# MLCogUP/nspeech

Measured on AMD Instinct MI355X. Metric: mel-frames/sec Tacotron-2 LJSpeech bs32 train step, higher is better.
Workload: dtype bf16; 1 GPU; Tacotron-2 train step (fwd+bwd+clip+Adam), batch 32/GPU, T_in 160, T_out 1000, r=5; targets = spectrogram features of synthetic speech (SURVEY 8d); global_batch=32, parallelism=dp1, deterministic_gradients=True

## Files before the change

include/nspeech_hip.h:

```cpp
#ifndef NSPEECH_HIP_H
#define NSPEECH_HIP_H
#include <stddef.h>
#include <stdint.h>

#ifdef __cplusplus
extern "C" {
#endif

typedef void* ns_stream_t;

enum { NS_OK = 0, NS_ERR_BAD_ARG = -1, NS_ERR_UNSUPPORTED_SHAPE = -2, NS_ERR_LAUNCH = -3,
       NS_ERR_SHORT_BUFFER = -4  };
enum { NS_F32 = 0, NS_BF16 = 1, NS_F64 = 2  };
enum { NS_ACT_NONE = 0, NS_ACT_RELU = 1, NS_ACT_TANH = 2, NS_ACT_SIGMOID = 3,
       NS_ACT_SOFTSIGN = 4  };

int ns_version(void);
const char* ns_device_arch(void);
const char* ns_last_error(void);

int ns_occupy(int blocks, int threads, int lds_bytes, int heavy, double usec, int* started, ns_stream_t stream);
int ns_wait_counter(const int* counter, int target, double timeout_usec, ns_stream_t stream);

typedef struct {
// ... 181 lines not shown
  int reverse;
  float forget_bias;
  void* h; int64_t ld_h;
  float* c;
  void* gates;
  const float* dh; int64_t ld_dh;
  void* dgates;
  float* work;
  int f32_passes;
  const void* whT_hi; const void* whT_lo; const void* wh_bf16;
  void* dgates_bf16;
  void* h_bf16; int64_t ld_h_bf16;
  uint32_t zoneout_thr_cell, zoneout_thr_output;
  uint32_t zoneout_seed_cell, zoneout_seed_output;
  float cell_clip;
} ns_lstm_seq_params;
int ns_lstm_seq_fwd(const ns_lstm_seq_params* p, ns_stream_t stream);
int ns_lstm_seq_bwd(const ns_lstm_seq_params* p, ns_stream_t stream);
size_t ns_lstm_seq_work_bytes(const ns_lstm_seq_params* p);
int ns_lstm_seq2_fwd(const ns_lstm_seq_params* p0, const ns_lstm_seq_params* p1, ns_stream_t stream);
int ns_lstm_seq2_bwd(const ns_lstm_seq_params* p0, const ns_lstm_seq_params* p1, ns_stream_t stream);


int ns_lstm_cluster_supported(const ns_lstm_seq_params* fw, const ns_lstm_seq_params* bw, int backward);
size_t ns_lstm_cluster_work_bytes(const ns_lstm_seq_params* p);
int ns_lstm_cluster_fwd(const ns_lstm_seq_params* fw, const ns_lstm_seq_params* bw, void* work, ns_stream_t stream);
int ns_lstm_cluster_bwd(const ns_lstm_seq_params* fw, const ns_lstm_seq_params* bw, void* work, ns_stream_t stream);

int ns_lstm_wide_supported(const ns_lstm_seq_params* p, int backward);
size_t ns_lstm_wide_work_bytes(const ns_lstm_seq_params* p);
// ... 369 lines not shown
```

nspeech_amd/csrc/lstm_wide.hip:

```cpp
#include "common.h"
#include <stdint.h>
#include <stdlib.h>

namespace {
constexpr int WT = 512, WW = WT / 64;
typedef unsigned int u32x4 __attribute__((ext_vector_type(4)));
constexpr size_t WIDE_TRACE_BYTES = 256 * 8 * sizeof(long long);

struct WideArgs {
  ns_lstm_seq_params p;
  int* status;
  long long* trace;
  int nub;
};
__device__ __forceinline__ void wstamp(const WideArgs& a, int st, int k) {
  if (a.trace && blockIdx.x == 0 && threadIdx.x == 0 && st < 256) a.trace[st * 8 + k] = wall_clock64();
}

template <typename T> __device__ __forceinline__ bool has_sentinel(const u32x4& v);
template <> __device__ __forceinline__ bool has_sentinel<float>(const u32x4& v) {
  return (v[0] == 0xffffffffu) | (v[1] == 0xffffffffu) | (v[2] == 0xffffffffu) | (v[3] == 0xffffffffu);
}
template <> __device__ __forceinline__ bool has_sentinel<bf16_t>(const u32x4& v) {
  bool b = false;
#pragma unroll
  for (int i = 0; i < 4; ++i) b = b | ((v[i] & 0xffffu) == 0xffffu) | (v[i] >= 0xffff0000u);
  return b;
}
__device__ __forceinline__ float clean(float x, float*) { return __float_as_uint(x) == 0xffffffffu ? __uint_as_float(0x7fc00000u) : x; }
__device__ __forceinline__ bf16_t clean(float x, bf16_t*) {
  const bf16_t b = (bf16_t)x;
  return __builtin_bit_cast(unsigned short, b) == 0xffffu ? __builtin_bit_cast(bf16_t, (unsigned short)0x7fc0u) : b;
}

template <typename T>
__global__ __launch_bounds__(256) void wide_fill_kernel(T* base, int N, long P, int padl, int T_, long ld, int width) {
  const int ppr = width * (int)sizeof(T) / 16;
  const long total = (long)N * T_ * ppr;
  const u32x4 s = {0xffffffffu, 0xffffffffu, 0xffffffffu, 0xffffffffu};
  for (long i = (long)blockIdx.x * blockDim.x + threadIdx.x; i < total; i += (long)gridDim.x * blockDim.x) {
    const long row = i / ppr;
    const int pc = (int)(i - row * ppr);
// ... 21 lines not shown
      ready |= __builtin_amdgcn_ballot_w64(lane < NP && !has_sentinel<T>(pv));
      if (tslot && ready == ALLP && blockIdx.x == 0 && threadIdx.x == 0) *tslot = wall_clock64();
    }
#pragma unroll
    for (int l = 0; l < NL; ++l) {
      constexpr unsigned long long one = 1ull;
      const unsigned long long m = ((one << PPCH) - one) << ((l / LPC) * PPCH);
      if (!(done & (1u << l)) && (ready & m) == m) {
        const unsigned o = off0 + (unsigned)(l % LPC) * in_grp + (unsigned)(l / LPC) * per_grp;
        v[l] = __builtin_amdgcn_raw_buffer_load_b128(rs, o, 0, 16);
        done |= 1u << l;
      }
    }
    ++spins;
    if (done == ALLL) {
      unsigned stale = 0u;
#pragma unroll
      for (int l = 0; l < NL; ++l) if (__any(has_sentinel<T>(v[l]))) stale |= 1u << l;
      if (!stale) return spins;
      done &= ~stale;
    }
    if ((spins & 255u) == 0) {
      if (__hip_atomic_load(status, __ATOMIC_RELAXED, __HIP_MEMORY_SCOPE_AGENT)) { if (lane == 0) *abortf = 1; return 0; }
      if ((spins & 1023u) == 0 && ns_spin_timed_out(clk0)) { if (lane == 0) { atomicExch(status, code); *abortf = 1; } return 0; }
    }
  }
}

constexpr int WTF = WT + 128;
template <typename T, int PASSES, int NCH>
__global__ __launch_bounds__(WTF) void lstm_wide_fwd_kernel(WideArgs a) {
  __shared__ float red[2][WW][16][36];
  __shared__ __attribute__((aligned(16))) T hst[16][8];
  __shared__ int abortf;
  const ns_lstm_seq_params& p = a.p;
  const int tid = threadIdx.x, lane = tid & 63, wave = __builtin_amdgcn_readfirstlane(tid >> 6);
  const int H = p.H, NUB = a.nub;
  const int rg = blockIdx.x / NUB, ub = blockIdx.x % NUB;
  const int n0 = rg * 16, u0 = ub * 8;
  if (tid == 0) abortf = 0;
  const size_t hbytes = (size_t)p.N * p.P * p.ld_h * sizeof(T);
  constexpr int PPC = 8 * (int)sizeof(T) / 16;
  __syncthreads();

  if (wave < WW) {
    const int r16 = lane & 15, g = lane >> 4;
    const int k0 = wave * (H / WW);
    bf16x8 bh[2][NCH], bl[2][NCH];
#pragma unroll
    for (int j = 0; j < 2; ++j) {
      const long wrow = ((long)(2 * j + (r16 >> 3)) * H + u0 + (r16 & 7)) * H + k0 + g * 8;
#pragma unroll
      for (int c = 0; c < NCH; ++c) {
        if constexpr (PASSES == 3) {
          bh[j][c] = *(const bf16x8*)((const bf16_t*)p.whT_hi + wrow + c * 32);
          bl[j][c] = *(const bf16x8*)((const bf16_t*)p.whT_lo + wrow + c * 32);
        } else {
          bh[j][c] = *(const bf16x8*)((const bf16_t*)p.whT + wrow + c * 32);
          bl[j][c] = bh[j][c];
        }
      }
    }
    const bool ok = n0 + r16 < p.N;
    const int prb = (ub * WW + wave) % min(16, p.N - n0);
    for (int t = 0; t < p.T; ++t) {
      f32x4 acc[2] = {{0.f, 0.f, 0.f, 0.f}, {0.f, 0.f, 0.f, 0.f}};
      wstamp(a, t, 0);
      if (t > 0) {
        const unsigned rowoff = ok ? (unsigned)(((long)(n0 + r16) * p.P + p.padl + t - 1) * p.ld_h + k0 + g * 8) * (unsigned)sizeof(T) : 0x80000000u;
        u32x4 v[NCH * PPC];
        const unsigned prow = (unsigned)(((long)(n0 + prb) * p.P + p.padl + t - 1) * p.ld_h + k0) * (unsigned)sizeof(T);
        const unsigned got = sweep_progressive<T, NCH * PPC, PPC, 4>(p.h, hbytes, prow, 8u * (unsigned)sizeof(T), rowoff, 16u, 32u * (unsigned)sizeof(T),
                                                                     v, lane, a.status, &abortf, 1, a.trace && t < 256 ? a.trace + t * 8 + 6 : nullptr);
        wstamp(a, t, 1);
        if (a.trace && blockIdx.x == 0 && tid == 0 && t < 256) a.trace[t * 8 + 5] = got;
        if (got) {
#pragma unroll
          for (int c = 0; c < NCH; ++c) {
            bf16x8 ah, al;
            if constexpr (sizeof(T) == 4) {
              const u32x4 x = v[2 * c], y = v[2 * c + 1];
              const float f[8] = {__uint_as_float(x[0]), __uint_as_float(x[1]), __uint_as_float(x[2]), __uint_as_float(x[3]),
                                  __uint_as_float(y[0]), __uint_as_float(y[1]), __uint_as_float(y[2]), __uint_as_float(y[3])};
#pragma unroll
              for (int i = 0; i < 8; ++i) { const bf16_t h = (bf16_t)f[i]; ah[i] = h; al[i] = (bf16_t)(f[i] - (float)h); }
            } else {
              ah = *(bf16x8*)&v[c];
              al = ah;
            }
#pragma unroll
            for (int j = 0; j < 2; ++j) {
              if constexpr (PASSES == 3) acc[j] = mfma_split<3>(ah, al, bh[j][c], bl[j][c], acc[j]);
              else acc[j] = __builtin_amdgcn_mfma_f32_16x16x32_bf16(ah, bh[j][c], acc[j], 0, 0, 0);
            }
          }
// ... 1 lines not shown
      }
#pragma unroll
      for (int j = 0; j < 2; ++j)
#pragma unroll
        for (int q = 0; q < 4; ++q) red[t & 1][wave][g * 4 + q][j * 16 + r16] = acc[j][q];
      __syncthreads();
      if (abortf) return;
      wstamp(a, t, 2);
    }
    return;
  }
  const int e = tid - WT, er = e >> 3, eu = e & 7;
  const int en = n0 + er;
  const bool eok = en < p.N;
  const int elen = (eok && p.lengths) ? p.lengths[en] : p.T;
  const auto hrs = __builtin_amdgcn_make_buffer_rsrc((void*)p.h, 0, (int)hbytes, 0x00020000);
  const bool tr = a.trace && blockIdx.x == 0 && e == 0;
  float cst = 0.f;
  float hprev = 0.f;
  const bool zone = p.zoneout_thr_cell != 0u || p.zoneout_thr_output != 0u;
  float pz[4] = {0.f, 0.f, 0.f, 0.f};
  auto load_xg = [&](int t) {
    if (eok) {
      const float* xr = p.xg + ((long)en * p.P + p.padl + t) * p.ld_xg + u0 + eu;
#pragma unroll
      for (int j = 0; j < 4; ++j) pz[j] = xr[(long)j * H];
    }
  };
  load_xg(0);
  for (int t = 0; t < p.T; ++t) {
    __syncthreads();
// ... 8 lines not shown
      z[j] = s;
    }
    float gi = sigmoidf_(z[0]), gj = tanhf_(z[1]), gf = sigmoidf_(z[2] + p.forget_bias), go = sigmoidf_(z[3]);
    float hv;
    if (!zone) {
      cst = ns_cell_clip(gf * cst + gi * gj, p.cell_clip);
      hv = go * tanhf_(cst);
    } else {
      const float cn = ns_cell_clip(gf * cst + gi * gj, p.cell_clip);
      hv = go * tanhf_(cn);
      if (!ns_zone_keep(p.zoneout_seed_cell, (uint32_t)t, (uint32_t)en, (uint32_t)(u0 + eu), p.zoneout_thr_cell)) cst = cn;
      if (ns_zone_keep(p.zoneout_seed_output, (uint32_t)t, (uint32_t)en, (uint32_t)(u0 + eu), p.zoneout_thr_output)) hv = hprev;
      hprev = hv;
    }
    if (t >= elen) { cst = 0.f; hv = 0.f; gi = gj = gf = go = 0.f; }
    hst[er][eu] = clean(hv, (T*)nullptr);
    __builtin_amdgcn_fence(__ATOMIC_RELEASE, "workgroup");
    __builtin_amdgcn_wave_barrier();
    if (lane < 8 * PPC) {
      const int row = (wave - WW) * 8 + lane / PPC, pc = lane % PPC;
      if (n0 + row < p.N) {
        const u32x4 x = *(const u32x4*)((const char*)&hst[row][0] + pc * 16);
        const unsigned off = (unsigned)(((long)(n0 + row) * p.P + p.padl + t) * p.ld_h + u0) * (unsigned)sizeof(T) + pc * 16;
        __builtin_amdgcn_raw_buffer_store_b128(x, hrs, off, 0, 16);
      }
    }
    if (tr && t < 256) a.trace[t * 8 + 4] = wall_clock64();
    if (eok) {
      const long rowi = (long)en * p.P + p.padl + t;
      p.c[rowi * H + u0 + eu] = cst;
      if (p.gates) {
        T* gp = (T*)p.gates + rowi * 4 * H + u0 + eu;
        stf(gp, gi); stf(gp + H, gj); stf(gp + 2 * H, gf); stf(gp + 3 * H, go);
      }
    }
    if (t + 1 < p.T) load_xg(t + 1);
  }
}

constexpr int PSW = 8;
constexpr int PST = PSW * 64 + 128;
typedef unsigned long long ps_u64;
__device__ __forceinline__ void ps_barrier() { asm volatile("s_waitcnt lgkmcnt(0)\n\ts_barrier" ::: "memory"); }

constexpr int UPB = 32;
template <typename T, int NT>
__global__ __launch_bounds__(PST) void lstm_wide_bwd_ps_kernel(WideArgs a, ps_u64* xbuf) {
  constexpr int TB = UPB / 16;
  constexpr int KO = 4 * UPB, KS = KO / 32;
  constexpr int ITEMS = UPB * 4;
  constexpr int IPL = ITEMS / 64;
  constexpr int LDW = KO + 8;
  constexpr int KSR = KS - 1;
  extern __shared__ __attribute__((aligned(16))) char ps_smem[];
  bf16_t* dgi = (bf16_t*)ps_smem;
  float* red = (float*)(dgi + 16 * LDW);
  float* ownp = red + PSW * ITEMS * 2;
  int* abortf = (int*)(ownp + ITEMS * 2);
  bf16x8* wl = (bf16x8*)(abortf + 4);
  const ns_lstm_seq_params& p = a.p;
  const int tid = threadIdx.x, lane = tid & 63, wave = __builtin_amdgcn_readfirstlane(tid >> 6);
// ... 66 lines not shown
      if (a.trace && blockIdx.x == 0 && tid == 0 && bs < 256) a.trace[bs * 8 + 5] = passes;
      if (a.trace && blockIdx.x == 0 && tid == 7 * 64 && bs < 256) a.trace[bs * 8 + 7] = wall_clock64();
#pragma unroll
      for (int i = 0; i < IPL; ++i) {
        red[((wave * ITEMS) + lane + 64 * i) * 2] = s0[i];
        red[((wave * ITEMS) + lane + 64 * i) * 2 + 1] = s1[i];
      }
      ps_barrier();
      wstamp(a, bs, 2);
      if (abortf[0]) return;
      ps_barrier();
      wstamp(a, bs, 3);
      if (bs + 1 < p.T) {
        bf16x8 af[KS];
#pragma unroll
        for (int ks = 0; ks < KS; ++ks) af[ks] = *(const bf16x8*)(dgi + r16 * LDW + 32 * ks + 8 * g);
        ps_u64* nxt = xb0 + (size_t)((bs + 1) & 1) * NUB * NUB * ITEMS;
        constexpr int TG = NT < 4 ? NT : 4;
#pragma unroll
        for (int j0 = 0; j0 < NT; j0 += TG) {
          f32x4 acc[TG];
#pragma unroll
          for (int jj = 0; jj < TG; ++jj) acc[jj] = (f32x4){0.f, 0.f, 0.f, 0.f};
#pragma unroll
          for (int ks = 0; ks < KS; ++ks)
#pragma unroll
            for (int jj = 0; jj < TG; ++jj)
              acc[jj] = __builtin_amdgcn_mfma_f32_16x16x32_bf16(af[ks], ks < KSR ? bw[j0 + jj][ks < KSR ? ks : 0] : wl[(wave * NT + j0 + jj) * 64 + lane],
                                                                acc[jj], 0, 0, 0);
#pragma unroll
          for (int jj = 0; jj < TG; ++jj) {
            const int tile = wave * NT + j0 + jj, dest = tile / TB, ui = (tile % TB) * 16 + r16;
            if (g < 2) {
              if (dest == ub) {
                ownp[(ui + UPB * (2 * g)) * 2] = acc[jj][0]; ownp[(ui + UPB * (2 * g)) * 2 + 1] = acc[jj][1];
                ownp[(ui + UPB * (2 * g + 1)) * 2] = acc[jj][2]; ownp[(ui + UPB * (2 * g + 1)) * 2 + 1] = acc[jj][3];
              } else {
                NS_GLOBAL ps_u64* dst = (NS_GLOBAL ps_u64*)(nxt + ((size_t)dest * NUB + ub) * ITEMS + ui + 2 * UPB * g);
                const ps_u64 tg = (ps_u64)(unsigned)(bs + 1) << 32;
                const bf16_t b0 = (bf16_t)acc[jj][0], b1 = (bf16_t)acc[jj][1], b2 = (bf16_t)acc[jj][2], b3 = (bf16_t)acc[jj][3];
                const unsigned p01 = (unsigned)__builtin_bit_cast(unsigned short, b0) | ((unsigned)__builtin_bit_cast(unsigned short, b1) << 16);
                const unsigned p23 = (unsigned)__builtin_bit_cast(unsigned short, b2) | ((unsigned)__builtin_bit_cast(unsigned short, b3) << 16);
                __hip_atomic_store(dst, tg | p01, __ATOMIC_RELAXED, __HIP_MEMORY_SCOPE_AGENT);
                __hip_atomic_store(dst + UPB, tg | p23, __ATOMIC_RELAXED, __HIP_MEMORY_SCOPE_AGENT);
              }
            }
          }
        }
      }
      wstamp(a, bs, 4);
    }
    return;
  }
  __syncthreads();
  const int e = tid - PSW * 64, er = e >> 4, eu = e & 15;
  const int en = n0 + er;
  const bool eok = en < p.N;
  const int elen = (eok && p.lengths) ? p.lengths[en] : p.T;
  const int half = er & 1;
// ... 89 lines not shown
    if (p->dtype == NS_BF16 && !p->wh) return false;
    if (!p->gates || !p->c || !p->dh || !p->dgates) return false;
    if (!al16(p->dtype == NS_BF16 ? p->dgates : p->dgates_bf16)) return false;
    if ((double)p->N * p->P * 4 * H * 2 >= 2.0e9) return false;
  }
  return true;
}

size_t ps_exchange_bytes(const ns_lstm_seq_params* p) {
  const size_t nb = p->H / UPB;
  return (size_t)((p->N + 7) / 8) * 2 * nb * nb * (UPB * 4) * sizeof(ps_u64);
}
}

extern "C" int ns_lstm_wide_supported(const ns_lstm_seq_params* p, int backward) { return wide_shape_ok(p, backward) ? 1 : 0; }
extern "C" size_t ns_lstm_wide_work_bytes(const ns_lstm_seq_params* p) {
  if (!p) return 0;
  const bool bwd_fits = (p->H == 256 || p->H == 512 || p->H == 1024) && (p->N + 15) / 16 * (p->H / 16) <= ns_device_cus();
  return 256 + WIDE_TRACE_BYTES + (bwd_fits ? ps_exchange_bytes(p) : 0) + 64;
}

template <typename T, int PASSES>
static int launch_wide_fwd(const WideArgs& a, int grid, hipStream_t s) {
  switch (a.p.H) {
    case 256: hipLaunchKernelGGL((lstm_wide_fwd_kernel<T, PASSES, 1>), dim3(grid), dim3(WTF), 0, s, a); break;
    case 512: hipLaunchKernelGGL((lstm_wide_fwd_kernel<T, PASSES, 2>), dim3(grid), dim3(WTF), 0, s, a); break;
    default: hipLaunchKernelGGL((lstm_wide_fwd_kernel<T, PASSES, 4>), dim3(grid), dim3(WTF), 0, s, a); break;
  }
  NS_CHECK_LAUNCH("lstm_wide_fwd");
  return NS_OK;
}

extern "C" int ns_lstm_wide_fwd(const ns_lstm_seq_params* p, void* work, ns_stream_t s_) {
  hipStream_t s = (hipStream_t)s_;
  NS_CHECK_ARG(p && work, "ns_lstm_wide_fwd: null");
  NS_CHECK_ARG(wide_shape_ok(p, 0), "ns_lstm_wide_fwd: unsupported (needs H in {256, 512, 1024}, row groups x H/8 <= 256, "
               "fp32 with pre-split whT_hi / whT_lo and f32_passes 3, or bf16)");
  WideArgs a;
  a.p = *p; a.status = (int*)work; a.nub = p->H / 8;
  a.trace = getenv("NS_WIDE_TRACE") ? (long long*)((char*)work + 256) : nullptr;
  int rc = ns_zero_async(work, 256, s);
  if (rc) return rc;
  const int grid = ((p->N + 15) / 16) * a.nub;
  if (p->dtype == NS_BF16) {
    hipLaunchKernelGGL(wide_fill_kernel<bf16_t>, dim3(512), dim3(256), 0, s, (bf16_t*)p->h, p->N, (long)p->P, p->padl, p->T, (long)p->ld_h, p->H);
    NS_CHECK_LAUNCH("lstm_wide_fill");
    return launch_wide_fwd<bf16_t, 1>(a, grid, s);
  }
  hipLaunchKernelGGL(wide_fill_kernel<float>, dim3(512), dim3(256), 0, s, (float*)p->h, p->N, (long)p->P, p->padl, p->T, (long)p->ld_h, p->H);
  NS_CHECK_LAUNCH("lstm_wide_fill");
  return launch_wide_fwd<float, 3>(a, grid, s);
}

typedef void (*wide_bwd_kernel_t)(WideArgs, ps_u64*);
#define NS_WIDE_BWD_FORMS(T_) {lstm_wide_bwd_ps_kernel<T_, 2>, lstm_wide_bwd_ps_kernel<T_, 4>, lstm_wide_bwd_ps_kernel<T_, 8>}
static const wide_bwd_kernel_t wide_bwd_forms[2][3] = {NS_WIDE_BWD_FORMS(bf16_t), NS_WIDE_BWD_FORMS(float)};
#undef NS_WIDE_BWD_FORMS

extern "C" int ns_lstm_wide_bwd(const ns_lstm_seq_params* p, void* work, ns_stream_t s_) {
  hipStream_t s = (hipStream_t)s_;
  NS_CHECK_ARG(p && work, "ns_lstm_wide_bwd: null");
  NS_CHECK_ARG(wide_shape_ok(p, 1), "ns_lstm_wide_bwd: unsupported (needs H in {256, 512, 1024}, row groups x H/16 <= 256, "
               "bf16, or fp32 with wh_bf16 + dgates_bf16 and f32_passes 1)");
  WideArgs a;
  a.p = *p; a.status = (int*)work; a.nub = 0;
  a.trace = getenv("NS_WIDE_TRACE") ? (long long*)((char*)work + 256) : nullptr;
  int rc = ns_zero_async(work, 256, s);
  if (rc) return rc;
  ps_u64* xbuf = (ps_u64*)(((uintptr_t)work + 256 + WIDE_TRACE_BYTES + 15) & ~(uintptr_t)15);
  rc = ns_zero_async(xbuf, ps_exchange_bytes(p), s);
  if (rc) return rc;
  const int grid = (p->N + 7) / 8 * (p->H / UPB);
  const int nt = p->H / 128, items = UPB * 4;
  const size_t ldsb = (size_t)16 * (4 * UPB + 8) * 2 + sizeof(float) * (PSW * items * 2 + items * 2) + 16 + (size_t)PSW * nt * 64 * 16;
  static bool attr = false;
  if (!attr) {
    for (const auto& widths : wide_bwd_forms)
      for (wide_bwd_kernel_t k : widths) (void)hipFuncSetAttribute((const void*)k, hipFuncAttributeMaxDynamicSharedMemorySize, 160 * 1024);
    attr = true;
  }
  hipLaunchKernelGGL(wide_bwd_forms[p->dtype == NS_BF16 ? 0 : 1][nt == 2 ? 0 : nt == 4 ? 1 : 2], dim3(grid), dim3(PST), ldsb, s, a, xbuf);
  NS_CHECK_LAUNCH("lstm_wide_bwd_ps");
  return NS_OK;
}
```

nspeech_amd/models/tacotron2.py:

```python
import math
import os

import numpy as np
import torch

from .. import ops
from .._lib import ACT_NONE, ACT_RELU, ACT_SOFTSIGN, ACT_TANH
from ..utils.text.symbols import symbols
from . import params as P_

PADL = 2
PADR = 2


def _round_up(x, m):
    return (x + m - 1) // m * m


class _LazyAudio(object):

    def __init__(self, model):
        self._m = model

    def __len__(self):
# ... 556 lines not shown
            Mg2 = rows - (k - 1) - a2
            ops.gemm(dpre, w16 if w16 is not None else self._W(D), dx, Mg2, cin, k * cout, cout, cout, cin, a_mode=0, b_mode=0,
                     a_off=a2 * cout, b_off=self._o(scope + "/conv1d/kernel") + (k - 1) * cin * cout,
                     b_seg=(cout, -cin * cout), c_off=self.padl * cin, accumulate=1 if dx_accumulate else 0,
                     row_mask=(Pp, self.padl, self.padl + T, self.padl), **self._dy_stats_kw(stats_for, self.padl))

    @staticmethod
    def _splitk(K, M, N):
        tiles = ((M + 127) // 128) * ((N + 127) // 128)
        sk = max(1, min(32, 512 // max(tiles, 1)))
        return max(1, min(sk, K // (256 if tiles <= 16 else 512)))

    def _x256_fits(self, rows, cout):
        return rows >= 1024 and ((rows + 255) // 256) * ((cout + 255) // 256) >= 96

    def _xg_gemm(self, x, xg, rows, cin, cout, key, woff, boff, D=None):
        D = D or self.T
        sh = self.tsh.get(key)
        if self._x256_fits(rows, cout) and D == torch.float32 and key + "_hi" in self.tsh:
            xh = self._buf("xgs_hi_" + key, rows * cin, torch.bfloat16)
            xl = self._buf("xgs_lo_" + key, rows * cin, torch.bfloat16)
            ops.split_hi_lo(x, xh, xl, rows * cin)
            ops.gemm(xh, self.tsh[key + "_hi"], xg, rows, cout, cin, cin, cin, cout, a_mode=0, b_mode=0, a_lo=xl,
                     b_lo=self.tsh[key + "_lo"], bias=self.flat_p, bias_off=boff)
        elif sh is not None and self._x256_fits(rows, cout) and D == torch.bfloat16 and sh.dtype == torch.bfloat16:
            ops.gemm(x, sh, xg, rows, cout, cin, cin, cin, cout, a_mode=0, b_mode=0, bias=self.flat_p, bias_off=boff)
        else:
            ops.gemm(x, self._W(D), xg, rows, cout, cin, cin, cout, cout, b_mode=1, b_off=woff, bias=self.flat_p, bias_off=boff)

    def _bilstm_fwd(self, scope, x, cin, H, N, T, Pp, lengths, tag, key, D=None):
        rows = N * Pp
        D = D or self.T
        out = self._buf(tag + "_h", rows * 2 * H, D)
        f32c = (D == torch.float32 and self.passes_fwd == 3 and self.use_cluster and H % 64 == 0 and H <= 256 and T >= 2
                and (self.passes_bwd == 1 or not self.is_training_pass))
        hb = self._buf(tag + "_h16", rows * 2 * H, torch.bfloat16) if f32c else None
        pair = []
# ... 24 lines not shown
            return None
        thr = ops.zoneout_threshold(self.zoneout_rate)
        base = self.zoneout_base_seed
        if torch.distributed.is_available() and torch.distributed.is_initialized():
            base ^= (torch.distributed.get_rank() * 0x9E3779B9) & 0xFFFFFFFF
        return (thr, thr, ops.zoneout_seed(base, self.global_step, 2 * layer),
                ops.zoneout_seed(base, self.global_step, 2 * layer + 1))

    def _run_lstm(self, direction, tag, *a, **kw):
        p = ops.lstm_seq_params(*a, **kw)
        if self.use_wide and ops.lstm_wide_supported(p, direction == "bwd"):
            w = self._buf("lstm_wide_work_%s_%s" % (tag, direction), ops.lstm_wide_work_floats(p), torch.float32)
            ops.lstm_wide(direction, p, w)
            self._status_words[(tag, direction)] = w
            self.last_paths["%s:%s" % (tag, direction)] = "wide"
        else:
            ops.lstm_seq_call(direction, p)
            self.last_paths["%s:%s" % (tag, direction)] = "step"

    use_cluster = True
    use_attn_cluster = True

    def _run_bilstm(self, direction, pair, tag):
        from .._lib import NS_BF16
        ok = pair[0].dtype == NS_BF16 or getattr(self, "_bilstm_f32c", {}).get(tag, False)
        if self.use_cluster and ok and ops.lstm_cluster_supported(pair[0], pair[1], direction == "bwd"):
            work = self._buf("lstm_cluster_work_%s_%s" % (tag, direction), ops.lstm_cluster_work_floats(pair[0]),
                             torch.float32)
            ops.lstm_cluster(direction, pair[0], pair[1], work)
            self._status_words[(tag, direction)] = work
            self.last_paths["%s:%s" % (tag, direction)] = "cluster"
        else:
            ops.lstm_seq2(direction, pair[0], pair[1])
# ... 190 lines not shown
            ops.taco2_attn_cluster("fwd", cw, **self._attn_args)
            self._status_words[("attn", "fwd")] = cw
        else:
            ops.taco2_attn("fwd", **self._attn_args)
        self.last_paths["attn:fwd"] = "cluster" if self._attn_cluster_fwd else "step"
        self._tick("attn_rnn")

        rows = N * S1
        k1, k2 = self._o("decoder/lstm_1/kernel"), self._o("decoder/lstm_2/kernel")
        xg1 = self._buf("dec_xg1", rows * 4 * D, torch.float32)
        self._xg_gemm(hc, xg1, rows, A + E, 4 * D, "l1_xT", k1, self._o("decoder/lstm_1/bias"))
        h1 = self._buf("dec_h1", rows * D, T_)
        c1 = self._buf("dec_c1", rows * D, torch.float32)
        g1 = self._buf("dec_g1", rows * 4 * D, T_)
        self._tick("dec_lstm:xg1")
        self._run_lstm("fwd", "dec1", N, S, D, S1, 1, xg1, 4 * D, self.tsh["l1_whT"], None, None, False, h1, D, c1, g1,
                       whT_hi=self.tsh.get("l1_whT_hi"), whT_lo=self.tsh.get("l1_whT_lo"), zoneout=self.zoneout_args(1))
        self._tick("dec_lstm:loop1")
        xg2 = self._buf("dec_xg2", rows * 4 * D, torch.float32)
        self._xg_gemm(h1, xg2, rows, D, 4 * D, "l2_xT", k2, self._o("decoder/lstm_2/bias"))
        h2 = self._buf("dec_h2", rows * D, T_)
        c2 = self._buf("dec_c2", rows * D, torch.float32)
        g2 = self._buf("dec_g2", rows * 4 * D, T_)
        self._tick("dec_lstm:xg2")
        self._run_lstm("fwd", "dec2", N, S, D, S1, 1, xg2, 4 * D, self.tsh["l2_whT"], None, None, False, h2, D, c2, g2,
                       whT_hi=self.tsh.get("l2_whT_hi"), whT_lo=self.tsh.get("l2_whT_lo"), zoneout=self.zoneout_args(2))
        self._tick("dec_lstm:loop2")
        dec = self._buf("dec_out", rows * M * r, torch.float32)
        ops.gemm(h2, self._W(self.T), dec, rows, M * r, D, D, M * r, M * r, b_mode=1,
                 b_off=self._o("decoder/output_projection/kernel"), bias=self.flat_p,
                 bias_off=self._o("decoder/output_projection/bias"))
        self._tick("dec_lstm")

        decp = self._buf("decp", N * Po * M, torch.float32)
        pin = self._buf("post_in", N * Po * M, T_)
        ops.copy3d(dec, decp, N, To, M, (S1 * M * r, M), (Po * M, M), src_off=M * r, dst_off=self.padl * M)
        ops.copy3d(dec, pin, N, To, M, (S1 * M * r, M), (Po * M, M), src_off=M * r, dst_off=self.padl * M)
        x = pin
        cin = M
        self._post_in = [x]
        Cp = hp.postnet_conv_channels
# ... 161 lines not shown
                       B["dec_c2"], B["dec_g2"], dh=dh2, ld_dh=D, dgates=dg2, work=work, wh_off=k2 + D * 4 * D,
                       wh_bf16=self._bf16_w(T_), wh_bf16_off=k2 + D * 4 * D,
                       dgates_bf16=self._dgb("d_g2b", rows * 4 * D, T_), zoneout=self.zoneout_args(2))
        self._tick("dec_lstm_bwd:loop2")
        w16 = self._bf16_w(T_)
        dg2b = self._bufs.get("d_g2b") if w16 is not None else None

        def b16(name, src, cols):
            return src if dg2b is None else self._buf(name, rows * cols, torch.bfloat16)

        def cast16(dst, src, cols):
            if dst is not src:
                ops.cast2d(src, rows, cols, cols, dst, cols, False)
        h1b, h2b = b16("dec_h1_16", h1, D), b16("dec_h2_16", h2, D)

        def lstm2_wgrads():
            cast16(h1b, h1, D)
            cast16(h2b, h2, D)
            self._lstm_wgrads(h1b, D, h2b, D, dg2b if dg2b is not None else dg2, rows, k2, "decoder/lstm_2/bias")
        self._defer("decoder", lstm2_wgrads, pure=True)
        if "decoder2" in self.queue_groups:
            self._flush_deferred()
        dh1 = self._buf("d_h1", rows * D, torch.float32)
        if dg2b is not None:
            ops.gemm(dg2b, w16, dh1, rows, D, 4 * D, 4 * D, 4 * D, D, a_mode=0, b_mode=0, b_off=k2)
        else:
            ops.gemm(dg2, self._W(self.T), dh1, rows, D, 4 * D, 4 * D, 4 * D, D, a_mode=0, b_mode=0, b_off=k2)
        dg1 = self._buf("d_g1", rows * 4 * D, T_)
        self._dgb("d_g1b", rows * 4 * D, T_)
        self._tick("dec_lstm_bwd:wgrad2")
        self._run_lstm("bwd", "dec1", N, S, D, S1, 1, B["dec_xg1"], 4 * D, None, self._W(self.T), None, False, h1, D,
                       B["dec_c1"], B["dec_g1"], dh=dh1, ld_dh=D, dgates=dg1, work=work, wh_off=k1 + (A + E) * 4 * D,
                       wh_bf16=self._bf16_w(T_), wh_bf16_off=k1 + (A + E) * 4 * D,
# ... 203 lines not shown
```

nspeech_amd/ops.py:

```python
import ctypes as C
import ctypes as C_

import torch

from . import _lib as L
from ._lib import NS_BF16, NS_F32


F32_PASSES = 0
CELL_CLIP = 0.0


def stream():
    return torch.cuda.current_stream().cuda_stream


def dt(t):
    if t.dtype == torch.float32:
        return NS_F32
    if t.dtype == torch.bfloat16:
        return NS_BF16
    raise TypeError("unsupported dtype %s" % t.dtype)


# ... 405 lines not shown
        raw = b"".join(bytes(p) for p in rec)
        self.table = torch.frombuffer(bytearray(raw), dtype=torch.uint8).to(self.device)
        self.ends = torch.tensor(ends, dtype=torch.int32, device=self.device)
        self.n, self.total = len(rec), tot
        return self

    def run(self):
        if self.n:
            L.check(L.lib().ns_cast2d_batch(C.c_void_p(self.table.data_ptr()), C.c_void_p(self.ends.data_ptr()), self.n,
                                            self.total, C.c_void_p(stream())), "ns_cast2d_batch")


def lstm_seq_params(N, T, H, P, padl, xg, ld_xg, whT, wh, lengths, reverse, h, ld_h, c, gates,
                    dh=None, ld_dh=0, dgates=None, work=None, xg_off=0, whT_off=0, wh_off=0, h_off=0, dh_off=0,
                    forget_bias=1.0, whT_hi=None, whT_lo=None, wh_bf16=None, wh_bf16_off=0, dgates_bf16=None,
                    h_bf16=None, h_bf16_off=0, ld_h_bf16=0, dtype=None, zoneout=None):
    p = L.struct("ns_lstm_seq_params")
    if zoneout is not None:
        p.zoneout_thr_cell, p.zoneout_thr_output, p.zoneout_seed_cell, p.zoneout_seed_output = [int(x) for x in zoneout]
    if h_bf16 is not None:
        p.h_bf16, p.ld_h_bf16 = ptr(h_bf16, h_bf16_off), ld_h_bf16
    _fill(p, dtype=dt(h) if dtype is None else dtype, N=N, T=T, H=H, P=P, padl=padl, xg=ptr(xg, xg_off), ld_xg=ld_xg,
          whT=ptr(whT, whT_off), wh=ptr(wh, wh_off), lengths=ptr(lengths), reverse=int(reverse),
          forget_bias=forget_bias, h=ptr(h, h_off), ld_h=ld_h, c=ptr(c), gates=ptr(gates),
          dh=ptr(dh, dh_off), ld_dh=ld_dh, dgates=ptr(dgates), work=ptr(work), f32_passes=F32_PASSES,
          whT_hi=ptr(whT_hi), whT_lo=ptr(whT_lo), wh_bf16=ptr(wh_bf16, wh_bf16_off), dgates_bf16=ptr(dgates_bf16),
          cell_clip=float(CELL_CLIP))
    return p


def zoneout_threshold(rate):
    return int(float(rate) * 16777216.0)
# ... 360 lines not shown
```

Baseline: 1.778 million mel-frames/s.

## Exchange pre-split bf16 hi/lo hidden states in wide LSTM forward and reuse them

In fp32 three-pass mode, the wide LSTM forward kernel now publishes each step's hidden state as bf16 hi/lo planes through a private exchange buffer. Consumers load these directly instead of fp32 values they must split per step. The same planes are written out, so the next layer's input GEMM can skip its split_hi_lo pass and the backward pass can skip the bf16 casts of h1/h2. The bwd exchange gains a lane-spread store layout (default on, env switch), and sentinel checks use packed u16 max. This costs extra workspace, more stores per step, and some code complexity.

```diff
diff --git a/include/nspeech_hip.h b/include/nspeech_hip.h
--- a/include/nspeech_hip.h
+++ b/include/nspeech_hip.h
@@ -219,6 +219,7 @@
   uint32_t zoneout_thr_cell, zoneout_thr_output;
   uint32_t zoneout_seed_cell, zoneout_seed_output;
   float cell_clip;
+  void* h_lo_bf16;
 } ns_lstm_seq_params;
 int ns_lstm_seq_fwd(const ns_lstm_seq_params* p, ns_stream_t stream);
 int ns_lstm_seq_bwd(const ns_lstm_seq_params* p, ns_stream_t stream);
diff --git a/nspeech_amd/csrc/lstm_wide.hip b/nspeech_amd/csrc/lstm_wide.hip
--- a/nspeech_amd/csrc/lstm_wide.hip
+++ b/nspeech_amd/csrc/lstm_wide.hip
@@ -12,6 +12,7 @@
   int* status;
   long long* trace;
   int nub;
+  void* xch;
 };
 __device__ __forceinline__ void wstamp(const WideArgs& a, int st, int k) {
   if (a.trace && blockIdx.x == 0 && threadIdx.x == 0 && st < 256) a.trace[st * 8 + k] = wall_clock64();
@@ -21,11 +22,13 @@
 template <> __device__ __forceinline__ bool has_sentinel<float>(const u32x4& v) {
   return (v[0] == 0xffffffffu) | (v[1] == 0xffffffffu) | (v[2] == 0xffffffffu) | (v[3] == 0xffffffffu);
 }
+typedef unsigned short u16x2 __attribute__((ext_vector_type(2)));
+__device__ __forceinline__ unsigned pk_max_u16(unsigned a, unsigned b) {
+  return __builtin_bit_cast(unsigned, __builtin_elementwise_max(__builtin_bit_cast(u16x2, a), __builtin_bit_cast(u16x2, b)));
+}
 template <> __device__ __forceinline__ bool has_sentinel<bf16_t>(const u32x4& v) {
-  bool b = false;
-#pragma unroll
-  for (int i = 0; i < 4; ++i) b = b | ((v[i] & 0xffffu) == 0xffffu) | (v[i] >= 0xffff0000u);
-  return b;
+  const unsigned m = pk_max_u16(pk_max_u16(v[0], v[1]), pk_max_u16(v[2], v[3]));
+  return ((m & 0xffffu) == 0xffffu) | (m >= 0xffff0000u);
 }
 __device__ __forceinline__ float clean(float x, float*) { return __float_as_uint(x) == 0xffffffffu ? __uint_as_float(0x7fc00000u) : x; }
 __device__ __forceinline__ bf16_t clean(float x, bf16_t*) {
@@ -77,6 +80,14 @@
     }
     ++spins;
     if (done == ALLL) {
+      if constexpr (sizeof(T) == 2) {
+        u32x4 m = v[0];
+#pragma unroll
+        for (int l = 1; l < NL; ++l)
+#pragma unroll
+          for (int i = 0; i < 4; ++i) m[i] = pk_max_u16(m[i], v[l][i]);
+        if (!__any(has_sentinel<T>(m))) return spins;
+      }
       unsigned stale = 0u;
 #pragma unroll
       for (int l = 0; l < NL; ++l) if (__any(has_sentinel<T>(v[l]))) stale |= 1u << l;
@@ -91,8 +102,9 @@
 }
 
 constexpr int WTF = WT + 128;
-template <typename T, int PASSES, int NCH>
+template <typename T, int PASSES, int NCH, bool SPLIT>
 __global__ __launch_bounds__(WTF) void lstm_wide_fwd_kernel(WideArgs a) {
+  static_assert(!SPLIT || (sizeof(T) == 4 && PASSES == 3), "the split form is the fp32 three-pass arrangement");
   __shared__ float red[2][WW][16][36];
   __shared__ __attribute__((aligned(16))) T hst[16][8];
   __shared__ int abortf;
@@ -102,7 +114,10 @@
   const int rg = blockIdx.x / NUB, ub = blockIdx.x % NUB;
   const int n0 = rg * 16, u0 = ub * 8;
   if (tid == 0) abortf = 0;
-  const size_t hbytes = (size_t)p.N * p.P * p.ld_h * sizeof(T);
+  const void* const xbase = SPLIT ? (const void*)a.xch : (const void*)p.h;
+  const long xld = SPLIT ? (long)p.H : (long)p.ld_h;
+  constexpr unsigned XSZ = (unsigned)sizeof(T);
+  const size_t hbytes = (size_t)p.N * p.P * xld * XSZ;
   constexpr int PPC = 8 * (int)sizeof(T) / 16;
   __syncthreads();
 
@@ -130,18 +145,25 @@
       f32x4 acc[2] = {{0.f, 0.f, 0.f, 0.f}, {0.f, 0.f, 0.f, 0.f}};
       wstamp(a, t, 0);
       if (t > 0) {
-        const unsigned rowoff = ok ? (unsigned)(((long)(n0 + r16) * p.P + p.padl + t - 1) * p.ld_h + k0 + g * 8) * (unsigned)sizeof(T) : 0x80000000u;
+        const unsigned rowoff = ok ? (unsigned)(((long)(n0 + r16) * p.P + p.padl + t - 1) * xld + k0 + g * 8) * XSZ : 0x80000000u;
         u32x4 v[NCH * PPC];
-        const unsigned prow = (unsigned)(((long)(n0 + prb) * p.P + p.padl + t - 1) * p.ld_h + k0) * (unsigned)sizeof(T);
-        const unsigned got = sweep_progressive<T, NCH * PPC, PPC, 4>(p.h, hbytes, prow, 8u * (unsigned)sizeof(T), rowoff, 16u, 32u * (unsigned)sizeof(T),
-                                                                     v, lane, a.status, &abortf, 1, a.trace && t < 256 ? a.trace + t * 8 + 6 : nullptr);
+        const unsigned prow = (unsigned)(((long)(n0 + prb) * p.P + p.padl + t - 1) * xld + k0) * XSZ;
+        long long* const tslot = a.trace && t < 256 ? a.trace + t * 8 + 6 : nullptr;
+        unsigned got;
+        if constexpr (SPLIT)
+          got = sweep_progressive<bf16_t, 2 * NCH, 2, 4>(xbase, hbytes, prow, 32u, rowoff, 16u, 128u, v, lane, a.status, &abortf, 1, tslot);
+        else
+          got = sweep_progressive<T, NCH * PPC, PPC, 4>(xbase, hbytes, prow, 8u * XSZ, rowoff, 16u, 32u * XSZ, v, lane, a.status, &abortf, 1, tslot);
         wstamp(a, t, 1);
         if (a.trace && blockIdx.x == 0 && tid == 0 && t < 256) a.trace[t * 8 + 5] = got;
         if (got) {
 #pragma unroll
           for (int c = 0; c < NCH; ++c) {
             bf16x8 ah, al;
-            if constexpr (sizeof(T) == 4) {
+            if constexpr (SPLIT) {
+              ah = *(bf16x8*)&v[2 * c];
+              al = *(bf16x8*)&v[2 * c + 1];
+            } else if constexpr (sizeof(T) == 4) {
               const u32x4 x = v[2 * c], y = v[2 * c + 1];
               const float f[8] = {__uint_as_float(x[0]), __uint_as_float(x[1]), __uint_as_float(x[2]), __uint_as_float(x[3]),
                                   __uint_as_float(y[0]), __uint_as_float(y[1]), __uint_as_float(y[2]), __uint_as_float(y[3])};
@@ -173,7 +195,7 @@
   const int en = n0 + er;
   const bool eok = en < p.N;
   const int elen = (eok && p.lengths) ? p.lengths[en] : p.T;
-  const auto hrs = __builtin_amdgcn_make_buffer_rsrc((void*)p.h, 0, (int)hbytes, 0x00020000);
+  const auto hrs = __builtin_amdgcn_make_buffer_rsrc((void*)xbase, 0, (int)hbytes, 0x00020000);
   const bool tr = a.trace && blockIdx.x == 0 && e == 0;
   float cst = 0.f;
   float hprev = 0.f;
@@ -212,20 +234,42 @@
       hprev = hv;
     }
     if (t >= elen) { cst = 0.f; hv = 0.f; gi = gj = gf = go = 0.f; }
-    hst[er][eu] = clean(hv, (T*)nullptr);
+    if constexpr (SPLIT) {
+      bf16_t* hsp = (bf16_t*)&hst[0][0];
+      const bf16_t hi = clean(hv, (bf16_t*)nullptr);
+      hsp[er * 8 + eu] = hi;
+      hsp[128 + er * 8 + eu] = clean(hv - (float)hi, (bf16_t*)nullptr);
+    } else {
+      hst[er][eu] = clean(hv, (T*)nullptr);
+    }
     __builtin_amdgcn_fence(__ATOMIC_RELEASE, "workgroup");
     __builtin_amdgcn_wave_barrier();
     if (lane < 8 * PPC) {
       const int row = (wave - WW) * 8 + lane / PPC, pc = lane % PPC;
       if (n0 + row < p.N) {
-        const u32x4 x = *(const u32x4*)((const char*)&hst[row][0] + pc * 16);
-        const unsigned off = (unsigned)(((long)(n0 + row) * p.P + p.padl + t) * p.ld_h + u0) * (unsigned)sizeof(T) + pc * 16;
-        __builtin_amdgcn_raw_buffer_store_b128(x, hrs, off, 0, 16);
+        if constexpr (SPLIT) {
+          const u32x4 x = *(const u32x4*)((const char*)&hst[0][0] + pc * 256 + row * 16);
+          const unsigned off = (unsigned)(((long)(n0 + row) * p.P + p.padl + t) * xld + u0) * XSZ + pc * 16;
+          __builtin_amdgcn_raw_buffer_store_b128(x, hrs, off, 0, 16);
+        } else {
+          const u32x4 x = *(const u32x4*)((const char*)&hst[row][0] + pc * 16);
+          const unsigned off = (unsigned)(((long)(n0 + row) * p.P + p.padl + t) * p.ld_h + u0) * (unsigned)sizeof(T) + pc * 16;
+          __builtin_amdgcn_raw_buffer_store_b128(x, hrs, off, 0, 16);
+        }
       }
     }
     if (tr && t < 256) a.trace[t * 8 + 4] = wall_clock64();
+    if constexpr (SPLIT) {
+      if (lane >= 16 && lane < 32) {
+        const int row = (wave - WW) * 8 + (lane - 16) / 2, pc = lane & 1;
+        if (n0 + row < p.N)
+          *(u32x4*)((bf16_t*)(pc ? p.h_lo_bf16 : p.h_bf16) + ((long)(n0 + row) * p.P + p.padl + t) * p.ld_h_bf16 + u0) =
+              *(const u32x4*)((const char*)&hst[0][0] + pc * 256 + row * 16);
+      }
+    }
     if (eok) {
       const long rowi = (long)en * p.P + p.padl + t;
+      if constexpr (SPLIT) ((float*)p.h)[rowi * p.ld_h + u0 + eu] = clean(hv, (float*)nullptr);
       p.c[rowi * H + u0 + eu] = cst;
       if (p.gates) {
         T* gp = (T*)p.gates + rowi * 4 * H + u0 + eu;
@@ -242,7 +286,7 @@
 __device__ __forceinline__ void ps_barrier() { asm volatile("s_waitcnt lgkmcnt(0)\n\ts_barrier" ::: "memory"); }
 
 constexpr int UPB = 32;
-template <typename T, int NT>
+template <typename T, int NT, bool LANES>
 __global__ __launch_bounds__(PST) void lstm_wide_bwd_ps_kernel(WideArgs a, ps_u64* xbuf) {
   constexpr int TB = UPB / 16;
   constexpr int KO = 4 * UPB, KS = KO / 32;
@@ -339,7 +383,7 @@
       if (bs + 1 < p.T) {
         bf16x8 af[KS];
 #pragma unroll
-        for (int ks = 0; ks < KS; ++ks) af[ks] = *(const bf16x8*)(dgi + r16 * LDW + 32 * ks + 8 * g);
+        for (int ks = 0; ks < KS; ++ks) af[ks] = *(const bf16x8*)(dgi + (LANES ? (r16 & 7) : r16) * LDW + 32 * ks + 8 * g);
         ps_u64* nxt = xb0 + (size_t)((bs + 1) & 1) * NUB * NUB * ITEMS;
         constexpr int TG = NT < 4 ? NT : 4;
 #pragma unroll
@@ -356,18 +400,29 @@
 #pragma unroll
           for (int jj = 0; jj < TG; ++jj) {
             const int tile = wave * NT + j0 + jj, dest = tile / TB, ui = (tile % TB) * 16 + r16;
-            if (g < 2) {
+            const ps_u64 tg = (ps_u64)(unsigned)(bs + 1) << 32;
+            auto granule = [&](float x0, float x1) {
+              const bf16_t b0 = (bf16_t)x0, b1 = (bf16_t)x1;
+              return tg | (ps_u64)((unsigned)__builtin_bit_cast(unsigned short, b0) | ((unsigned)__builtin_bit_cast(unsigned short, b1) << 16));
+            };
+            if constexpr (LANES) {
+              const int gp = g & 1, hf = g >> 1;
+              const float x0 = hf ? acc[jj][2] : acc[jj][0], x1 = hf ? acc[jj][3] : acc[jj][1];
+              const int item = ui + UPB * (2 * gp + hf);
+              if (dest == ub) {
+                ownp[item * 2] = x0; ownp[item * 2 + 1] = x1;
+              } else {
+                __hip_atomic_store((NS_GLOBAL ps_u64*)(nxt + ((size_t)dest * NUB + ub) * ITEMS + item), granule(x0, x1), __ATOMIC_RELAXED,
+                                   __HIP_MEMORY_SCOPE_AGENT);
+              }
+            } else if (g < 2) {
               if (dest == ub) {
                 ownp[(ui + UPB * (2 * g)) * 2] = acc[jj][0]; ownp[(ui + UPB * (2 * g)) * 2 + 1] = acc[jj][1];
                 ownp[(ui + UPB * (2 * g + 1)) * 2] = acc[jj][2]; ownp[(ui + UPB * (2 * g + 1)) * 2 + 1] = acc[jj][3];
               } else {
                 NS_GLOBAL ps_u64* dst = (NS_GLOBAL ps_u64*)(nxt + ((size_t)dest * NUB + ub) * ITEMS + ui + 2 * UPB * g);
-                const ps_u64 tg = (ps_u64)(unsigned)(bs + 1) << 32;
-                const bf16_t b0 = (bf16_t)acc[jj][0], b1 = (bf16_t)acc[jj][1], b2 = (bf16_t)acc[jj][2], b3 = (bf16_t)acc[jj][3];
-                const unsigned p01 = (unsigned)__builtin_bit_cast(unsigned short, b0) | ((unsigned)__builtin_bit_cast(unsigned short, b1) << 16);
-                const unsigned p23 = (unsigned)__builtin_bit_cast(unsigned short, b2) | ((unsigned)__builtin_bit_cast(unsigned short, b3) << 16);
-                __hip_atomic_store(dst, tg | p01, __ATOMIC_RELAXED, __HIP_MEMORY_SCOPE_AGENT);
-                __hip_atomic_store(dst + UPB, tg | p23, __ATOMIC_RELAXED, __HIP_MEMORY_SCOPE_AGENT);
+                __hip_atomic_store(dst, granule(acc[jj][0], acc[jj][1]), __ATOMIC_RELAXED, __HIP_MEMORY_SCOPE_AGENT);
+                __hip_atomic_store(dst + UPB, granule(acc[jj][2], acc[jj][3]), __ATOMIC_RELAXED, __HIP_MEMORY_SCOPE_AGENT);
               }
             }
           }
@@ -487,18 +542,24 @@
 }
 
 extern "C" int ns_lstm_wide_supported(const ns_lstm_seq_params* p, int backward) { return wide_shape_ok(p, backward) ? 1 : 0; }
+static size_t wide_work_base(const ns_lstm_seq_params* p) {
+  const bool bwd_fits = (p->H == 256 || p->H == 512 || p->H == 1024) && (p->N + 15) / 16 * (p->H / 16) <= ns_device_cus();
+  return 256 + WIDE_TRACE_BYTES + (bwd_fits ? ps_exchange_bytes(p) : 0) + 64;
+}
+static void* wide_xch(const ns_lstm_seq_params* p, void* work) {
+  return (void*)(((uintptr_t)work + wide_work_base(p) + 255) & ~(uintptr_t)255);
+}
 extern "C" size_t ns_lstm_wide_work_bytes(const ns_lstm_seq_params* p) {
   if (!p) return 0;
-  const bool bwd_fits = (p->H == 256 || p->H == 512 || p->H == 1024) && (p->N + 15) / 16 * (p->H / 16) <= ns_device_cus();
-  return 256 + WIDE_TRACE_BYTES + (bwd_fits ? ps_exchange_bytes(p) : 0) + 64;
-}
-
-template <typename T, int PASSES>
+  return wide_work_base(p) + ((p->h_bf16 && p->h_lo_bf16) ? 256 + (size_t)p->N * p->P * p->H * 4 : 0);
+}
+
+template <typename T, int PASSES, bool SPLIT>
 static int launch_wide_fwd(const WideArgs& a, int grid, hipStream_t s) {
   switch (a.p.H) {
-    case 256: hipLaunchKernelGGL((lstm_wide_fwd_kernel<T, PASSES, 1>), dim3(grid), dim3(WTF), 0, s, a); break;
-    case 512: hipLaunchKernelGGL((lstm_wide_fwd_kernel<T, PASSES, 2>), dim3(grid), dim3(WTF), 0, s, a); break;
-    default: hipLaunchKernelGGL((lstm_wide_fwd_kernel<T, PASSES, 4>), dim3(grid), dim3(WTF), 0, s, a); break;
+    case 256: hipLaunchKernelGGL((lstm_wide_fwd_kernel<T, PASSES, 1, SPLIT>), dim3(grid), dim3(WTF), 0, s, a); break;
+    case 512: hipLaunchKernelGGL((lstm_wide_fwd_kernel<T, PASSES, 2, SPLIT>), dim3(grid), dim3(WTF), 0, s, a); break;
+    default: hipLaunchKernelGGL((lstm_wide_fwd_kernel<T, PASSES, 4, SPLIT>), dim3(grid), dim3(WTF), 0, s, a); break;
   }
   NS_CHECK_LAUNCH("lstm_wide_fwd");
   return NS_OK;
@@ -507,10 +568,18 @@
 extern "C" int ns_lstm_wide_fwd(const ns_lstm_seq_params* p, void* work, ns_stream_t s_) {
   hipStream_t s = (hipStream_t)s_;
   NS_CHECK_ARG(p && work, "ns_lstm_wide_fwd: null");
+  NS_CHECK_ARG(!p->h_lo_bf16 || p->h_bf16, "ns_lstm_wide_fwd: h_lo_bf16 without h_bf16 (the lo plane goes with the hi plane)");
+  const bool split = p->dtype == NS_F32 && p->f32_passes == 3 && p->h_bf16 && p->h_lo_bf16;
   NS_CHECK_ARG(wide_shape_ok(p, 0), "ns_lstm_wide_fwd: unsupported (needs H in {256, 512, 1024}, row groups x H/8 <= 256, "
                "fp32 with pre-split whT_hi / whT_lo and f32_passes 3, or bf16)");
+  if (split) {
+    NS_CHECK_ARG(p->ld_h_bf16 >= p->H && p->ld_h_bf16 % 8 == 0 && ((uintptr_t)p->h_bf16 & 15) == 0 && ((uintptr_t)p->h_lo_bf16 & 15) == 0,
+                 "ns_lstm_wide_fwd: h_bf16 / h_lo_bf16 need 16-byte alignment and ld_h_bf16 %% 8 == 0, >= H");
+    NS_CHECK_ARG((double)p->N * p->P * p->H * 4 < 2.0e9, "ns_lstm_wide_fwd: exchange array beyond a buffer resource");
+  }
   WideArgs a;
   a.p = *p; a.status = (int*)work; a.nub = p->H / 8;
+  a.xch = split ? wide_xch(p, work) : nullptr;
   a.trace = getenv("NS_WIDE_TRACE") ? (long long*)((char*)work + 256) : nullptr;
   int rc = ns_zero_async(work, 256, s);
   if (rc) return rc;
@@ -518,16 +587,22 @@
   if (p->dtype == NS_BF16) {
     hipLaunchKernelGGL(wide_fill_kernel<bf16_t>, dim3(512), dim3(256), 0, s, (bf16_t*)p->h, p->N, (long)p->P, p->padl, p->T, (long)p->ld_h, p->H);
     NS_CHECK_LAUNCH("lstm_wide_fill");
-    return launch_wide_fwd<bf16_t, 1>(a, grid, s);
+    return launch_wide_fwd<bf16_t, 1, false>(a, grid, s);
+  }
+  if (split) {
+    hipLaunchKernelGGL(wide_fill_kernel<float>, dim3(512), dim3(256), 0, s, (float*)a.xch, p->N, (long)p->P, p->padl, p->T, (long)p->H, p->H);
+    NS_CHECK_LAUNCH("lstm_wide_fill");
+    return launch_wide_fwd<float, 3, true>(a, grid, s);
   }
   hipLaunchKernelGGL(wide_fill_kernel<float>, dim3(512), dim3(256), 0, s, (float*)p->h, p->N, (long)p->P, p->padl, p->T, (long)p->ld_h, p->H);
   NS_CHECK_LAUNCH("lstm_wide_fill");
-  return launch_wide_fwd<float, 3>(a, grid, s);
+  return launch_wide_fwd<float, 3, false>(a, grid, s);
 }
 
 typedef void (*wide_bwd_kernel_t)(WideArgs, ps_u64*);
-#define NS_WIDE_BWD_FORMS(T_) {lstm_wide_bwd_ps_kernel<T_, 2>, lstm_wide_bwd_ps_kernel<T_, 4>, lstm_wide_bwd_ps_kernel<T_, 8>}
-static const wide_bwd_kernel_t wide_bwd_forms[2][3] = {NS_WIDE_BWD_FORMS(bf16_t), NS_WIDE_BWD_FORMS(float)};
+#define NS_WIDE_BWD_FORMS(T_, L_) {lstm_wide_bwd_ps_kernel<T_, 2, L_>, lstm_wide_bwd_ps_kernel<T_, 4, L_>, lstm_wide_bwd_ps_kernel<T_, 8, L_>}
+static const wide_bwd_kernel_t wide_bwd_forms[2][2][3] = {{NS_WIDE_BWD_FORMS(bf16_t, false), NS_WIDE_BWD_FORMS(float, false)},
+                                                          {NS_WIDE_BWD_FORMS(bf16_t, true), NS_WIDE_BWD_FORMS(float, true)}};
 #undef NS_WIDE_BWD_FORMS
 
 extern "C" int ns_lstm_wide_bwd(const ns_lstm_seq_params* p, void* work, ns_stream_t s_) {
@@ -536,7 +611,7 @@
   NS_CHECK_ARG(wide_shape_ok(p, 1), "ns_lstm_wide_bwd: unsupported (needs H in {256, 512, 1024}, row groups x H/16 <= 256, "
                "bf16, or fp32 with wh_bf16 + dgates_bf16 and f32_passes 1)");
   WideArgs a;
-  a.p = *p; a.status = (int*)work; a.nub = 0;
+  a.p = *p; a.status = (int*)work; a.nub = 0; a.xch = nullptr;
   a.trace = getenv("NS_WIDE_TRACE") ? (long long*)((char*)work + 256) : nullptr;
   int rc = ns_zero_async(work, 256, s);
   if (rc) return rc;
@@ -548,11 +623,14 @@
   const size_t ldsb = (size_t)16 * (4 * UPB + 8) * 2 + sizeof(float) * (PSW * items * 2 + items * 2) + 16 + (size_t)PSW * nt * 64 * 16;
   static bool attr = false;
   if (!attr) {
-    for (const auto& widths : wide_bwd_forms)
-      for (wide_bwd_kernel_t k : widths) (void)hipFuncSetAttribute((const void*)k, hipFuncAttributeMaxDynamicSharedMemorySize, 160 * 1024);
+    for (const auto& lanes : wide_bwd_forms)
+      for (const auto& widths : lanes)
+        for (wide_bwd_kernel_t k : widths) (void)hipFuncSetAttribute((const void*)k, hipFuncAttributeMaxDynamicSharedMemorySize, 160 * 1024);
     attr = true;
   }
-  hipLaunchKernelGGL(wide_bwd_forms[p->dtype == NS_BF16 ? 0 : 1][nt == 2 ? 0 : nt == 4 ? 1 : 2], dim3(grid), dim3(PST), ldsb, s, a, xbuf);
+  const char* le = getenv("NS_WIDE_LANES");
+  const int lanes = (le && le[0] == '0' && !le[1]) ? 0 : 1;
+  hipLaunchKernelGGL(wide_bwd_forms[lanes][p->dtype == NS_BF16 ? 0 : 1][nt == 2 ? 0 : nt == 4 ? 1 : 2], dim3(grid), dim3(PST), ldsb, s, a, xbuf);
   NS_CHECK_LAUNCH("lstm_wide_bwd_ps");
   return NS_OK;
 }
diff --git a/nspeech_amd/models/tacotron2.py b/nspeech_amd/models/tacotron2.py
--- a/nspeech_amd/models/tacotron2.py
+++ b/nspeech_amd/models/tacotron2.py
@@ -594,13 +594,16 @@
     def _x256_fits(self, rows, cout):
         return rows >= 1024 and ((rows + 255) // 256) * ((cout + 255) // 256) >= 96
 
-    def _xg_gemm(self, x, xg, rows, cin, cout, key, woff, boff, D=None):
+    def _xg_gemm(self, x, xg, rows, cin, cout, key, woff, boff, D=None, presplit=None):
         D = D or self.T
         sh = self.tsh.get(key)
         if self._x256_fits(rows, cout) and D == torch.float32 and key + "_hi" in self.tsh:
-            xh = self._buf("xgs_hi_" + key, rows * cin, torch.bfloat16)
-            xl = self._buf("xgs_lo_" + key, rows * cin, torch.bfloat16)
-            ops.split_hi_lo(x, xh, xl, rows * cin)
+            if presplit is not None:
+                xh, xl = presplit
+            else:
+                xh = self._buf("xgs_hi_" + key, rows * cin, torch.bfloat16)
+                xl = self._buf("xgs_lo_" + key, rows * cin, torch.bfloat16)
+                ops.split_hi_lo(x, xh, xl, rows * cin)
             ops.gemm(xh, self.tsh[key + "_hi"], xg, rows, cout, cin, cin, cin, cout, a_mode=0, b_mode=0, a_lo=xl,
                      b_lo=self.tsh[key + "_lo"], bias=self.flat_p, bias_off=boff)
         elif sh is not None and self._x256_fits(rows, cout) and D == torch.bfloat16 and sh.dtype == torch.bfloat16:
@@ -655,9 +658,16 @@
             ops.lstm_wide(direction, p, w)
             self._status_words[(tag, direction)] = w
             self.last_paths["%s:%s" % (tag, direction)] = "wide"
-        else:
-            ops.lstm_seq_call(direction, p)
-            self.last_paths["%s:%s" % (tag, direction)] = "step"
+            return True
+        ops.lstm_seq_call(direction, p)
+        self.last_paths["%s:%s" % (tag, direction)] = "step"
+        return False
+
+    def _h_planes(self, name, rows, D):
+        if self.mode != "mixed" or not self.use_wide:
+            return None, None
+        b = self._buf(name, 2 * rows * D, torch.bfloat16)
+        return b, b[rows * D:]
 
     use_cluster = True
     use_attn_cluster = True
@@ -878,17 +888,23 @@
         c1 = self._buf("dec_c1", rows * D, torch.float32)
         g1 = self._buf("dec_g1", rows * 4 * D, T_)
         self._tick("dec_lstm:xg1")
-        self._run_lstm("fwd", "dec1", N, S, D, S1, 1, xg1, 4 * D, self.tsh["l1_whT"], None, None, False, h1, D, c1, g1,
-                       whT_hi=self.tsh.get("l1_whT_hi"), whT_lo=self.tsh.get("l1_whT_lo"), zoneout=self.zoneout_args(1))
+        h1hi, h1lo = self._h_planes("dec_h1_16", rows, D)
+        wide1 = self._run_lstm("fwd", "dec1", N, S, D, S1, 1, xg1, 4 * D, self.tsh["l1_whT"], None, None, False, h1, D, c1, g1,
+                               whT_hi=self.tsh.get("l1_whT_hi"), whT_lo=self.tsh.get("l1_whT_lo"), zoneout=self.zoneout_args(1),
+                               h_bf16=h1hi, ld_h_bf16=D, h_lo_bf16=h1lo)
         self._tick("dec_lstm:loop1")
         xg2 = self._buf("dec_xg2", rows * 4 * D, torch.float32)
-        self._xg_gemm(h1, xg2, rows, D, 4 * D, "l2_xT", k2, self._o("decoder/lstm_2/bias"))
+        self._xg_gemm(h1, xg2, rows, D, 4 * D, "l2_xT", k2, self._o("decoder/lstm_2/bias"),
+                      presplit=(h1hi, h1lo) if (wide1 and h1hi is not None) else None)
         h2 = self._buf("dec_h2", rows * D, T_)
         c2 = self._buf("dec_c2", rows * D, torch.float32)
         g2 = self._buf("dec_g2", rows * 4 * D, T_)
         self._tick("dec_lstm:xg2")
-        self._run_lstm("fwd", "dec2", N, S, D, S1, 1, xg2, 4 * D, self.tsh["l2_whT"], None, None, False, h2, D, c2, g2,
-                       whT_hi=self.tsh.get("l2_whT_hi"), whT_lo=self.tsh.get("l2_whT_lo"), zoneout=self.zoneout_args(2))
+        h2hi, h2lo = self._h_planes("dec_h2_16", rows, D)
+        wide2 = self._run_lstm("fwd", "dec2", N, S, D, S1, 1, xg2, 4 * D, self.tsh["l2_whT"], None, None, False, h2, D, c2, g2,
+                               whT_hi=self.tsh.get("l2_whT_hi"), whT_lo=self.tsh.get("l2_whT_lo"), zoneout=self.zoneout_args(2),
+                               h_bf16=h2hi, ld_h_bf16=D, h_lo_bf16=h2lo)
+        self._h16_written = (wide1 and h1hi is not None, wide2 and h2hi is not None)
         self._tick("dec_lstm:loop2")
         dec = self._buf("dec_out", rows * M * r, torch.float32)
         ops.gemm(h2, self._W(self.T), dec, rows, M * r, D, D, M * r, M * r, b_mode=1,
@@ -1080,9 +1096,13 @@
                 ops.cast2d(src, rows, cols, cols, dst, cols, False)
         h1b, h2b = b16("dec_h1_16", h1, D), b16("dec_h2_16", h2, D)
 
+        h1_done, h2_done = getattr(self, "_h16_written", (False, False))
+
         def lstm2_wgrads():
-            cast16(h1b, h1, D)
-            cast16(h2b, h2, D)
+            if not h1_done:
+                cast16(h1b, h1, D)
+            if not h2_done:
+                cast16(h2b, h2, D)
             self._lstm_wgrads(h1b, D, h2b, D, dg2b if dg2b is not None else dg2, rows, k2, "decoder/lstm_2/bias")
         self._defer("decoder", lstm2_wgrads, pure=True)
         if "decoder2" in self.queue_groups:
diff --git a/nspeech_amd/ops.py b/nspeech_amd/ops.py
--- a/nspeech_amd/ops.py
+++ b/nspeech_amd/ops.py
@@ -443,8 +443,10 @@
 def lstm_seq_params(N, T, H, P, padl, xg, ld_xg, whT, wh, lengths, reverse, h, ld_h, c, gates,
                     dh=None, ld_dh=0, dgates=None, work=None, xg_off=0, whT_off=0, wh_off=0, h_off=0, dh_off=0,
                     forget_bias=1.0, whT_hi=None, whT_lo=None, wh_bf16=None, wh_bf16_off=0, dgates_bf16=None,
-                    h_bf16=None, h_bf16_off=0, ld_h_bf16=0, dtype=None, zoneout=None):
+                    h_bf16=None, h_bf16_off=0, ld_h_bf16=0, dtype=None, zoneout=None, h_lo_bf16=None, h_lo_bf16_off=0):
     p = L.struct("ns_lstm_seq_params")
+    if h_lo_bf16 is not None:
+        p.h_lo_bf16 = ptr(h_lo_bf16, h_lo_bf16_off)
     if zoneout is not None:
         p.zoneout_thr_cell, p.zoneout_thr_output, p.zoneout_seed_cell, p.zoneout_seed_output = [int(x) for x in zoneout]
     if h_bf16 is not None:
```

New measurement: 1.797 million mel-frames/s, median of 6. 1.01x the previous value.
